# philres/ngmlr

Hardware: AMD Instinct MI355X
Metric: aligned Gbp/hour (PacBio 10kb synthetic, convex-gap SW hot path, host buffers in -> results out, CIGAR bit-exact) (higher is better)
Workload: dtype f32

## Files before the change

### ngmlr_amd/csrc/cvx_host_logic.h

```cpp
#ifndef CVX_HOST_LOGIC_H
#define CVX_HOST_LOGIC_H

#include <algorithm>
#include <atomic>
#include <cmath>
#include <condition_variable>
#include <cstdlib>
#include <cstring>
#include <deque>
#include <functional>
#include <mutex>
#include <system_error>
#include <thread>
#include <vector>

#include <pthread.h>

#include "cvx_align.h"
#include "cvx_types.h"

namespace cvx {


struct KernelClass {
// ... 700 lines not shown
				continue;
			}
		} else {
			ring = kClasses[k].ring();
		}
		r.ring = (int32_t) ring;
		r.r0 = p.r0;
		r.nsteps = p.rend - p.r0;
		r.dir_off = hp.dir_dwords;
		hp.dir_dwords += (uint64_t) ((r.nsteps + 31) / 32) * (uint64_t) r.ring * 2ull;
		r.mnw = k < 0 ? 0 : kClasses[k].m;
		if (k < 0) { hp.generic.push_back(i); continue; }
		hp.n_fast++;
		hp.cls[(size_t) k * 2 + (wrap ? 1 : 0)].push_back(i);
	}
	for (size_t slot = 0; slot < per_tile.size(); ++slot) {
		size_t deepest = 0;
		for (auto &v : per_tile[slot]) deepest = std::max(deepest, v.size());
		for (size_t g = 0; g < deepest; ++g)
			for (auto &v : per_tile[slot])
				if (g < v.size()) hp.chain_tasks[slot].push_back(v[g]);
	}
	for (auto &v : hp.cls) lpt_sort(v, plan);
}



struct ScheduleTuning {
	int exact_steps = kExactDirectSteps;
	int bt_group = 0;
	bool bt_per_class = true;
	bool overlap_post = false;
	int wide_prio = 1, gang_prio = 0, chain_prio = -1, chain_lds_kb = 48;
};

enum { kModeTwoPhase = 0, kModeExact = 1, kModeChain = 2 };

enum StreamSlot { kOnSide0 = 0, kOnPost = 1, kOnMain = 2, kOnSide1 = 3, kStreamSlots = 4 };

struct WalkPlan { int n_long = 0, long_lanes = 32, bulk_lanes = 64; };

inline WalkPlan walk_plan(int count, int n_walk, int bt_group, uint64_t mean_h, const int32_t *list, const TileIn *tin) {
	const int auto_group = count <= 6144 ? 64 : count <= 12288 ? 32 : count <= 49152 ? 16 : 8;
	WalkPlan w;
	w.bulk_lanes = bt_group > 0 ? bt_group : bt_group < 0 ? (n_walk < 4096 ? 64 : 8) : auto_group;
	if (bt_group <= 0 && w.bulk_lanes <= 16)
		while (w.n_long < count && (uint64_t) tin[(size_t) list[w.n_long]].H > 3 * mean_h) w.n_long++;
	return w;
}

inline size_t chain_pad_lds(uint64_t live, int num_cus, int chain_lds_kb, bool rings_beside) {
	const uint64_t resident = std::min<uint64_t>(8192, std::max<uint64_t>(768, live + live / 2 + 256));
	const size_t per_cu = (size_t) ((resident + (uint64_t) num_cus - 1) / (uint64_t) num_cus);
	size_t pad_lds = per_cu >= 32 ? 0 : (size_t) (160 * 1024) / per_cu - 4096;
	pad_lds = std::min<size_t>(pad_lds, 60 * 1024) / 256 * 256;
	if (rings_beside && chain_lds_kb > 0 && per_cu > 0 && per_cu < 32) {
		const size_t budget = (size_t) chain_lds_kb * 1024 / per_cu;
		const size_t capped = budget > 4096 ? (budget - 4096) / 256 * 256 : 0;
		pad_lds = std::min(pad_lds, capped);
	}
	return pad_lds;
}

struct FillLaunch {
	int kind = 0;
	int m = 0, gang = 1, wrap = 0;
	int slot = 0;
	const std::vector<int32_t> *tiles = nullptr;
	size_t list_off = 0;
	int n_direct = 0, count = 0;
	size_t pad_lds = 0;
	int prio = 0;
	int stream = kOnMain;
	size_t bt_off = 0;
	int bt_count = 0;
	WalkPlan walk;
	cvx_launch_info info;
};

struct ComputeSchedule {
	std::vector<FillLaunch> launches;
	size_t n_listed = 0;
	size_t bt_begin = 0;
	int n_walk = 0;
	bool per_class = false;
	WalkPlan walk;
	size_t chain_task_off[kNumChainClasses * 2] = {0}, chain_tile_off[kNumChainClasses * 2] = {0};
	size_t chain_blk_off = 0, chain_bytes = 0;
};

inline void build_schedule(HostPlan &hp, const TilePlan *plan, const TileIn *tin, int n, uint64_t n_rows, int num_cus,
		const ScheduleTuning &t, int32_t *lists, ComputeSchedule &s) {
	size_t n_listed = 0;
	size_t cls_off[kNumClasses * 2];
	int n_direct[kNumClasses * 2];
	int ring_classes = 0;
	for (size_t c = 0; c < hp.cls.size(); ++c) {
		std::vector<int32_t> &v = hp.cls[c];
		cls_off[c] = n_listed;
		n_direct[c] = 0;
		if (v.empty()) continue;
		ring_classes++;
		auto direct = [&](int32_t ti) { return hp.trun[(size_t) ti].nsteps >= t.exact_steps; };
		const int nl = t.exact_steps > 0 ? (int) std::count_if(v.begin(), v.end(), direct) : 0;
		if (nl > 0 && nl <= kExactDirectMaxTiles) {
			std::stable_partition(v.begin(), v.end(), direct);
			for (int q = 0; q < nl; ++q) hp.tout[(size_t) v[(size_t) q]].pad = kPadRedo;
			n_direct[c] = nl;
		}
		memcpy(lists + n_listed, v.data(), v.size() * sizeof(int32_t));
		n_listed += v.size();
	}
	const size_t generic_begin = n_listed;
	if (!hp.generic.empty()) memcpy(lists + n_listed, hp.generic.data(), hp.generic.size() * sizeof(int32_t));
	n_listed += hp.generic.size();

	s.launches.clear();
	s.launches.reserve((size_t) (kNumChainClasses + kNumClasses) * 2 + 1);
	for (size_t c = 0; c < hp.chain_tasks.size(); ++c) {
		if (hp.chain_tasks[c].empty()) continue;
		FillLaunch L;
		L.kind = CVX_LAUNCH_CHAINED;
		L.m = kChainClasses[c / 2]; L.wrap = (int) (c & 1); L.slot = (int) c;
		L.tiles = &hp.chain_tiles[c];
		L.count = (int) hp.chain_tasks[c].size();
		L.prio = t.chain_prio >= 0 ? t.chain_prio : 1;
		uint64_t live = 0;
		for (int32_t ti : hp.chain_tiles[c]) live += (uint64_t) plan[(size_t) ti].need / (uint64_t) (64 * L.m + kChainChunk) + 2;
		L.pad_lds = chain_pad_lds(live, num_cus, t.chain_lds_kb, ring_classes > 0);
		s.launches.push_back(L);
	}
	bool widest = true;
	for (int cc = (int) hp.cls.size() - 1; cc >= 0; --cc) {
		const size_t c = (size_t) cc;
		if (hp.cls[c].empty()) continue;
		const KernelClass &kc = kClasses[c / 2];
		FillLaunch L;
		L.kind = kc.gang > 1 ? CVX_LAUNCH_GANG : CVX_LAUNCH_WHOLE;
		L.m = kc.m; L.gang = kc.gang; L.wrap = (int) (c & 1); L.slot = cc;
		L.tiles = &hp.cls[c];
		L.list_off = cls_off[c]; L.n_direct = n_direct[c]; L.count = (int) hp.cls[c].size();
		L.prio = kc.gang > 1 ? t.gang_prio : (widest && ring_classes > 1) ? t.wide_prio : 0;
		widest = false;
		s.launches.push_back(L);
	}
	if (!hp.generic.empty()) {
		FillLaunch L;
		L.kind = CVX_LAUNCH_CATCH_ALL;
		L.m = 0; L.gang = 16; L.wrap = 1;
		L.tiles = &hp.generic;
		L.list_off = generic_begin; L.count = (int) hp.generic.size();
		s.launches.push_back(L);
	}

	int order[kStreamSlots], n_order = 0;
	for (int sl = 0; sl < kStreamSlots; ++sl) if (sl != kOnPost || !t.overlap_post) order[n_order++] = sl;
	s.bt_begin = n_listed;
	constexpr int kBuckets = 4096;
	auto bucket = [&](int32_t ti) { const int k = tin[(size_t) ti].H >> 5; return kBuckets - 1 - (k < kBuckets ? k : kBuckets - 1); };
	std::vector<int32_t> count((size_t) kBuckets + 1);
	for (size_t i = 0; i < s.launches.size(); ++i) {
		FillLaunch &L = s.launches[i];
		L.stream = order[i % (size_t) n_order];
		memset(&L.info, 0, sizeof(L.info));
		L.info.slots_per_lane = L.m; L.info.wrap16 = L.wrap; L.info.n_tiles = (int) L.tiles->size(); L.info.kind = L.kind;
		L.info.waves = L.kind == CVX_LAUNCH_CHAINED ? L.count : L.gang;
		std::fill(count.begin(), count.end(), 0);
		for (int32_t ti : *L.tiles) {
			const TilePlan &p = plan[(size_t) ti];
			const TileIn &in = tin[(size_t) ti];
			L.info.cells += p.cells; L.info.active_cells += p.active;
			L.info.alg_bytes += p.cells + 6ull * (uint64_t) in.H + 2ull * (uint64_t) in.W;
			L.info.read_bases += (uint64_t) in.H;
			if (!hp.trun[(size_t) ti].skip) count[(size_t) bucket(ti) + 1]++;
		}
		for (int k = 0; k < kBuckets; ++k) count[(size_t) k + 1] += count[(size_t) k];
		L.bt_off = n_listed;
		L.bt_count = count[(size_t) kBuckets];
		for (int32_t ti : *L.tiles) if (!hp.trun[(size_t) ti].skip) lists[n_listed + (size_t) count[(size_t) bucket(ti)]++] = ti;
		n_listed += (size_t) L.bt_count;
	}
	s.n_listed = n_listed;
	s.n_walk = (int) (n_listed - s.bt_begin);

	s.per_class = t.bt_per_class && s.launches.size() > 1 && !t.overlap_post && s.n_walk >= 4096;
	const uint64_t mean_h = n_rows / (uint64_t) std::max(n, 1);
	if (s.per_class) for (FillLaunch &L : s.launches) L.walk = walk_plan(L.bt_count, s.n_walk, t.bt_group, mean_h, lists + L.bt_off, tin);
	else s.walk = walk_plan(s.n_walk, s.n_walk, t.bt_group, mean_h, lists + s.bt_begin, tin);

	s.chain_blk_off = s.chain_bytes = 0;
	if (hp.n_chained) {
		for (size_t c = 0; c < hp.chain_tasks.size(); ++c) { s.chain_task_off[c] = s.chain_bytes; s.chain_bytes += hp.chain_tasks[c].size() * sizeof(ChainTask); }
		s.chain_blk_off = s.chain_bytes; s.chain_bytes += hp.chain_blk.size() * sizeof(ChainBlk);
		for (size_t c = 0; c < hp.chain_tiles.size(); ++c) { s.chain_tile_off[c] = s.chain_bytes; s.chain_bytes += (hp.chain_tiles[c].size() * sizeof(int32_t) + 7) / 8 * 8; }
	}
}

}

#endif
```

### ngmlr_amd/csrc/cvx_rt.h

```cpp
#ifndef CVX_RT_H
#define CVX_RT_H

#include <hip/hip_runtime_api.h>

#include <atomic>
#include <cstdint>
#include <mutex>
#include <string>
#include <vector>

#include "cvx_align.h"
#include "cvx_host_logic.h"
#include "cvx_launch.h"
#include "cvx_nm_regions.h"
#include "cvx_rt_err.h"
#include "cvx_types.h"

using namespace cvx;

#define HIP_TRY(expr)                                                              \
	do {                                                                           \
		hipError_t e_ = (expr);                                                    \
		if (e_ != hipSuccess) {                                                    \
			set_err("%s failed: %s (%s:%d)", #expr, hipGetErrorString(e_), __FILE__, __LINE__); \
// ... 86 lines not shown
			want = asked;
			e = hipHostMalloc(&p, want, hipHostMallocDefault);
		}
		if (e != hipSuccess) {
			(void) hipGetLastError();
			set_err("hipHostMalloc(%zu bytes) failed: %s", want, hipGetErrorString(e));
			p = nullptr;
			return CVX_ERR_OOM;
		}
		cap = want;
		if (hwm && cap > *hwm) *hwm = cap;
		return CVX_OK;
	}
	void release() {
		if (p) (void) hipHostFree(p);
		p = nullptr;
		cap = 0;
	}
	template <typename T> T *as() const { return static_cast<T *>(p); }
};

bool in_pinned_block(const void *p, uint64_t bytes);
float ev_ms(hipEvent_t a, hipEvent_t b);
int ensure_streams(cvx_context *c);
void search_state_free(cvx_search_state *ss);
float search_kernel_ms(const cvx_search_state *ss);
float search_score_kernel_ms(const cvx_search_state *ss);
void score_state_free(cvx_score_state *ss);

}

static const int kAuxStreams = 2;

enum LaunchEvent { kLevStart = 0, kLevTwoPhase = 1, kLevExact = 2, kLevWalked = 3, kLevPerLaunch = 4 };

enum BatchState { kFailed = -1, kEmpty = 0, kUploaded = 1, kPlanned = 2, kComputed = 3, kFinished = 4 };

struct cvx_batch_s {
	int n = 0;
	int state = kEmpty;
	bool in_flight = false;
	hipStream_t s_run = nullptr;
	int fail_rc = CVX_OK;
	std::string fail_msg;
	uint64_t seq_total = 0, n_rows = 0, n_rowsx = 0;
	uint64_t zero_copy_bytes = 0;
	uint64_t ops_total = 0;
	uint64_t dense_cap = 0;
	bool have_ops = false;

	PinBuf h_zero;
	size_t zero_cap = 0;
	PinBuf h_seq, h_delta, h_rsrc, h_rowsx, h_tin;
	std::vector<RowDesc> chain_rows;
	PinBuf h_plan;
	PinBuf h_trun, h_tout, h_lists, h_goff;
	PinBuf h_res;
	PinBuf h_ops;

	DevBuf<uint8_t> d_seq;
	DevBuf<RowDesc> d_rows;
	DevBuf<uint8_t> d_delta;
	DevBuf<RowSrc> d_rsrc;
	DevBuf<RowDesc> d_rowsx;
	DevBuf<TileIn> d_tin;
	DevBuf<TilePlan> d_plan;
	DevBuf<TileRun> d_trun;
// ... 14 lines not shown
	DevBuf<uint8_t> d_text;
	bool text_done = false;
	DevBuf<unsigned long long> d_nmoff;
	DevBuf<int32_t> d_nm;
	PinBuf h_nmoff;
	PinBuf h_nm;
	hipEvent_t ev_nm0 = nullptr, ev_nm1 = nullptr;
	DevBuf<unsigned long long> d_nmroff;
	DevBuf<NmOpen> d_nmopen;
	DevBuf<NmRegion> d_nmstage;
	DevBuf<NmRegion> d_nmreg;
	PinBuf h_nmroff, h_nmopen;
	PinBuf h_nmreg;
	PinBuf h_win;
	PinBuf h_refs;
	uint64_t refs_base = 0;
	bool have_refs = false;
	DevBuf<WindowDesc> d_win;
	PinBuf h_reads;
	PinBuf h_segs;
	DevBuf<uint8_t> d_reads, d_segs;
	PinBuf h_chain;
	DevBuf<uint8_t> d_chain;
	DevBuf<BoundaryRec> d_bnd;
	uint32_t bnd_epoch = 0;
	DevBuf<ChainOut> d_chain_out;

	hipEvent_t ev_bt0 = nullptr, ev_bt1 = nullptr;
	hipEvent_t ev_in = nullptr;
	hipEvent_t ev_res = nullptr;
	hipEvent_t ev[5] = {nullptr, nullptr, nullptr, nullptr, nullptr};
	std::vector<hipEvent_t> lev;
	std::vector<cvx_launch_info> launches;
	cvx_timing timing;

	const TileIn *tin() const { return h_tin.as<TileIn>(); }
	const TilePlan *plan() const { return h_plan.as<TilePlan>(); }
	const ResultRec *res() const { return h_res.as<ResultRec>(); }
	const BatchSummary *summary() const { return reinterpret_cast<const BatchSummary *>(h_res.as<uint8_t>() + (size_t) n * sizeof(ResultRec)); }

	static const int kSharedMarks = 40;
	void bind(size_t *marks) {
		int k = 0;
		PinBuf *pins[] = { &h_seq, &h_delta, &h_rsrc, &h_tin, &h_plan, &h_trun, &h_tout, &h_lists, &h_res, &h_ops, &h_chain };
		for (PinBuf *b_ : pins) b_->hwm = &marks[k++];
		d_seq.hwm = &marks[k++]; d_rows.hwm = &marks[k++]; d_delta.hwm = &marks[k++]; d_rsrc.hwm = &marks[k++]; d_tin.hwm = &marks[k++];
		d_plan.hwm = &marks[k++]; d_trun.hwm = &marks[k++]; d_tout.hwm = &marks[k++]; d_dirs.hwm = &marks[k++]; d_regions.hwm = &marks[k++];
		d_lists.hwm = &marks[k++]; d_dstoff.hwm = &marks[k++]; d_dense.hwm = &marks[k++]; d_res.hwm = &marks[k++];
		d_chain.hwm = &marks[k++]; d_bnd.hwm = &marks[k++]; d_chain_out.hwm = &marks[k++];
		h_text.hwm = &marks[k++]; h_nm.hwm = &marks[k++]; d_text.hwm = &marks[k++]; d_nm.hwm = &marks[k++];
		h_reads.hwm = &marks[k++]; h_segs.hwm = &marks[k++]; d_reads.hwm = &marks[k++]; d_segs.hwm = &marks[k++];
		static_assert(11 + 17 + 4 + 4 <= kSharedMarks, "marks");
	}
	int make_events() {
		if (!ev_in) HIP_TRY(hipEventCreateWithFlags(&ev_in, hipEventDisableTiming));
		if (!ev_res) HIP_TRY(hipEventCreateWithFlags(&ev_res, hipEventDisableTiming));
		if (!ev_bt0) HIP_TRY(hipEventCreateWithFlags(&ev_bt0, hipEventDisableTiming));
		if (!ev_bt1) HIP_TRY(hipEventCreateWithFlags(&ev_bt1, hipEventDisableTiming));
		for (auto &e : ev) if (!e) HIP_TRY(hipEventCreate(&e));
		return CVX_OK;
	}
	void release() {
		h_zero.release(); zero_cap = 0;
		h_seq.release(); h_delta.release(); h_rsrc.release(); h_rowsx.release(); h_tin.release();
		d_delta.release(); d_rsrc.release(); d_rowsx.release(); h_plan.release(); h_trun.release(); h_tout.release();
		h_lists.release(); h_goff.release(); h_res.release(); h_ops.release();
		d_seq.release(); d_rows.release(); d_tin.release(); d_plan.release(); d_trun.release();
		d_tout.release(); d_dirs.release(); d_regions.release(); d_lists.release();
		d_counters.release(); d_dstoff.release(); d_dense.release(); d_res.release();
		d_gscratch.release(); d_gscratch_off.release();
		h_win.release(); d_win.release(); h_refs.release();
		h_reads.release(); h_segs.release(); d_reads.release(); d_segs.release();
		h_ext.release(); h_trec.release(); h_toff.release(); h_text.release();
		d_ext.release(); d_trec.release(); d_tlen.release(); d_text.release();
		d_nmoff.release(); d_nm.release(); h_nmoff.release(); h_nm.release();
		d_nmroff.release(); d_nmopen.release(); d_nmstage.release(); d_nmreg.release(); h_nmroff.release(); h_nmopen.release(); h_nmreg.release();
		if (ev_nm0) { (void) hipEventDestroy(ev_nm0); ev_nm0 = nullptr; }
		if (ev_nm1) { (void) hipEventDestroy(ev_nm1); ev_nm1 = nullptr; }
		h_chain.release(); d_chain.release(); d_bnd.release(); d_chain_out.release();
		if (ev_in) { (void) hipEventDestroy(ev_in); ev_in = nullptr; }
		if (ev_res) { (void) hipEventDestroy(ev_res); ev_res = nullptr; }
		if (ev_bt0) { (void) hipEventDestroy(ev_bt0); ev_bt0 = nullptr; }
		if (ev_bt1) { (void) hipEventDestroy(ev_bt1); ev_bt1 = nullptr; }
		for (auto &e : ev) if (e) { (void) hipEventDestroy(e); e = nullptr; }
		for (auto &e : lev) if (e) (void) hipEventDestroy(e);
		lev.clear();
	}
};

struct cvx_context {
	int device = 0;
	hipStream_t s_io = nullptr;
	hipStream_t s_main = nullptr;
	hipStream_t s_text = nullptr;
	hipStream_t s_post = nullptr;
	hipStream_t aux[kAuxStreams] = {nullptr};
	bool service = false;
	bool owns_main = true;
	std::mutex streams_mtx;
	std::atomic<bool> streams_ready{false};
	hipStream_t s_main2 = nullptr, s_post2 = nullptr, aux2[kAuxStreams] = {nullptr};
	unsigned small_jobs = 0;
	ScoreParams sp;
	uint64_t max_matrix_mb = 10000;
	int num_cus = 256;
	int pack_threads = 16;
	int tune_min_slots = 0;
	int tune_late_min = kLateMinGroups;
	int tune_late_shift = kLateShift;
	int tune_max_slots = 0;
	int tune_long_need = 0;
	int tune_gang_prio = 0;
	int tune_gangs = 0;
	int tune_long_steps = 0, tune_small_batch = 0;
	bool single_lane = true;
	int tune_exact_steps = kExactDirectSteps;
	int tune_wide_prio = 1;
	int tune_chain_prio = -1;
	int tune_chain_lds_kb = 48;
	int tune_chain_m = 0;
	int tune_force_wrap = 0;
	int tune_pen_table = 1;
	int test_fail_compute = 0;
	int bt_group = 0;
	bool bt_per_class = true;
	bool overlap_post = false;
	bool scalar_twin = false;
	bool force_generic = false;
	bool sse_variant = false;
	size_t marks[cvx_batch_s::kSharedMarks] = {0};
	std::vector<cvx_batch_s *> pool;
	std::vector<cvx_batch_s *> pending;
	std::vector<cvx_batch_s *> live;
	float segments_kernel_ms = 0.0f;
	float decode_kernel_ms = 0.0f;
	bool score_no_diag = false;
	struct cvx_score_state *score = nullptr;
	struct cvx_search_state *search = nullptr;
};

struct cvx_genome_s {
	int device = 0;
	uint64_t n_nibbles = 0;
	int32_t n_starts = 0;
	DevBuf<uint8_t> d_bin;
	DevBuf<uint64_t> d_starts;
};

#endif
```

### ngmlr_amd/csrc/cvx_rt_align.cpp

```cpp
#include <algorithm>
#include <atomic>
#include <chrono>
#include <cstdio>
#include <cstdlib>
#include <cstring>
#include <new>
#include <string>
#include <vector>

#include "cvx_qry_stage.h"
#include "cvx_rt.h"

namespace {

struct SegmentsIn {
	int32_t n_reads;
	const uint8_t *arena;
	const uint64_t *offsets;
	const cvx_read_segment *qry;
};

static const size_t kPoolBatches = 8;

cvx_batch_s *acquire_batch(cvx_context *h) {
	if (!h->pool.empty()) {
		cvx_batch_s *b = h->pool.back();
		h->pool.pop_back();
		return b;
	}
	return new (std::nothrow) cvx_batch_s();
}

void recycle_batch(cvx_context *h, cvx_batch_s *b) {
	const bool failed = b->state == kFailed;
	b->state = kEmpty;
	b->in_flight = false;
	b->have_ops = false;
	b->have_refs = false;
	b->text_done = false;
	b->fail_rc = CVX_OK;
	b->fail_msg.clear();
	if (h) {
// ... 236 lines not shown
		if (!hp.chain_tasks[c].empty()) memcpy(hc + sch.chain_task_off[c], hp.chain_tasks[c].data(), hp.chain_tasks[c].size() * sizeof(ChainTask));
	memcpy(hc + sch.chain_blk_off, hp.chain_blk.data(), hp.chain_blk.size() * sizeof(ChainBlk));
	for (size_t c = 0; c < hp.chain_tiles.size(); ++c)
		if (!hp.chain_tiles[c].empty()) memcpy(hc + sch.chain_tile_off[c], hp.chain_tiles[c].data(), hp.chain_tiles[c].size() * sizeof(int32_t));
	RC_TRY(b->d_chain.ensure(sch.chain_bytes));
	RC_TRY(b->d_chain_out.ensure(hp.chain_blk.size()));
	{
		const size_t had = b->d_bnd.cap;
		RC_TRY(b->d_bnd.ensure((size_t) hp.bnd_recs + 64));
		if (b->d_bnd.cap != had || b->bnd_epoch >= kBndEpochMax) {
			HIP_TRY(hipMemsetAsync(b->d_bnd.p, 0, b->d_bnd.cap * sizeof(BoundaryRec), st));
			b->bnd_epoch = 0;
		}
		b->bnd_epoch += 1;
	}
	HIP_TRY(hipMemcpyAsync(b->d_chain.p, hc, sch.chain_bytes, hipMemcpyHostToDevice, st));
	return CVX_OK;
}

int stage_compute(cvx_context *h, cvx_batch_s *b, bool streaming = false) {
	const int n = b->n;
	if (h->test_fail_compute > 0 && --h->test_fail_compute == 0) {
		set_err("stage_compute: failure injected by CVX_TUNE_FAIL_COMPUTE");
		return CVX_ERR_OOM;
	}
	const bool second = streaming && n > 0 && n < kSmallJobTiles && !h->single_lane && ((h->small_jobs++ & 1u) != 0u);
	hipStream_t const S_main = second ? h->s_main2 : h->s_main;
	hipStream_t const S_post = second ? h->s_post2 : h->s_post;
	hipStream_t const *S_aux = second ? h->aux2 : h->aux;
	b->s_run = S_main;
	hipStream_t st = S_main;
	HIP_TRY(hipEventSynchronize(b->ev_in));
	b->launches.clear();
	b->ops_total = 0;
	b->have_ops = false;
	if (n == 0) {
		HIP_TRY(hipEventRecord(b->ev[4], st));
		hipStream_t ps = h->overlap_post ? S_post : S_main;
		HIP_TRY(hipStreamWaitEvent(ps, b->ev[4], 0));
		HIP_TRY(hipEventRecord(b->ev[2], ps));
		HIP_TRY(hipEventRecord(b->ev[3], ps));
		HIP_TRY(hipEventRecord(b->ev_res, ps));
		b->state = kComputed;
		return CVX_OK;
	}

	HostPlan hp;
	PlanTuning tune;
	tune.min_slots = h->tune_min_slots; tune.max_slots = h->tune_max_slots; tune.force_wrap = h->tune_force_wrap; tune.chain_m = h->tune_chain_m;
	tune.force_generic = h->force_generic ? 1 : 0;
	tune.long_steps = h->tune_long_steps; tune.small_batch = h->tune_small_batch; tune.long_need = h->tune_long_need;
	tune.no_gangs = h->tune_gangs ? 0 : 1;
	const RowSrc *rsrc = b->h_rsrc.as<RowSrc>();
	host_plan_rows(n, b->plan(), b->tin(), [&](int i, std::vector<RowDesc> &tmp) -> const RowDesc * {
		tmp.resize((size_t) std::max(b->tin()[(size_t) i].H, 1));
		expand_rows_host(rsrc[(size_t) i], b->tin()[(size_t) i].H, b->h_delta.as<uint8_t>(), b->h_rowsx.as<RowDesc>(), tmp.data());
		return tmp.data();
	}, true, tune, hp);
	const std::vector<int32_t> &generic = hp.generic;
	RC_TRY(b->d_dirs.ensure((size_t) hp.dir_dwords + 64));
	RC_TRY(b->d_regions.ensure((size_t) hp.ops_ints + 64));
	b->dense_cap = std::min<uint64_t>(hp.ops_ints, hp.ops_ints / 3 + 64ull * (uint64_t) n);
	RC_TRY(b->d_dense.ensure((size_t) b->dense_cap + 64));
	b->dense_cap = std::max<uint64_t>(b->dense_cap, b->d_dense.cap - 64);

	RC_TRY(b->h_trun.ensure((size_t) n * sizeof(TileRun)));
	RC_TRY(b->h_tout.ensure((size_t) n * sizeof(TileOut)));
	RC_TRY(b->h_lists.ensure((size_t) 2 * n * sizeof(int32_t) + 64));
	ScheduleTuning stune;
	stune.exact_steps = h->tune_exact_steps; stune.bt_group = h->bt_group; stune.bt_per_class = h->bt_per_class; stune.overlap_post = h->overlap_post;
	stune.wide_prio = h->tune_wide_prio; stune.gang_prio = h->tune_gang_prio; stune.chain_prio = h->tune_chain_prio; stune.chain_lds_kb = h->tune_chain_lds_kb;
	ComputeSchedule sch;
	build_schedule(hp, b->plan(), b->tin(), n, b->n_rows, h->num_cus, stune, b->h_lists.as<int32_t>(), sch);
	memcpy(b->h_trun.p, hp.trun.data(), (size_t) n * sizeof(TileRun));
	memcpy(b->h_tout.p, hp.tout.data(), (size_t) n * sizeof(TileOut));
	if (!generic.empty()) {
		RC_TRY(b->h_goff.ensure((generic.size() + 1) * sizeof(uint64_t)));
		uint64_t *goff = b->h_goff.as<uint64_t>();
		goff[0] = 0;
		for (size_t g = 0; g < generic.size(); ++g)
			goff[g + 1] = goff[g] + (uint64_t) generic_scratch_bytes(hp.trun[(size_t) generic[g]].ring);
		RC_TRY(b->d_gscratch.ensure((size_t) goff[generic.size()] + 256));
		RC_TRY(b->d_gscratch_off.ensure(generic.size() + 1));
		HIP_TRY(hipMemcpyAsync(b->d_gscratch_off.p, goff, (generic.size() + 1) * sizeof(uint64_t), hipMemcpyHostToDevice, st));
	}
	if (hp.n_chained) RC_TRY(upload_chain(b, hp, sch, st));
	HIP_TRY(hipMemcpyAsync(b->d_trun.p, b->h_trun.p, (size_t) n * sizeof(TileRun), hipMemcpyHostToDevice, st));
	HIP_TRY(hipMemcpyAsync(b->d_tout.p, b->h_tout.p, (size_t) n * sizeof(TileOut), hipMemcpyHostToDevice, st));
	if (sch.n_listed) HIP_TRY(hipMemcpyAsync(b->d_lists.p, b->h_lists.p, sch.n_listed * sizeof(int32_t), hipMemcpyHostToDevice, st));
	HIP_TRY(hipEventRecord(b->ev[4], st));

	FillArgs fa;
	BacktrackArgs ba;
	kernel_args(h, b, hp.n_chained ? reinterpret_cast<const ChainBlk *>(b->d_chain.p + sch.chain_blk_off) : nullptr, fa, ba);
	static_assert(kAuxStreams == 2, "StreamSlot names two side streams");
	hipStream_t fill_streams[kStreamSlots];
	fill_streams[kOnSide0] = S_aux[0]; fill_streams[kOnPost] = S_post; fill_streams[kOnMain] = st; fill_streams[kOnSide1] = S_aux[1];
	const int launches = (int) sch.launches.size();
	while (b->lev.size() < (size_t) launches * kLevPerLaunch) {
		hipEvent_t e;
		HIP_TRY(hipEventCreate(&e));
		b->lev.push_back(e);
	}
	for (int i = 0; i < launches; ++i) {
		const FillLaunch &L = sch.launches[(size_t) i];
		const hipStream_t ls = fill_streams[L.stream];
		const hipEvent_t *le = &b->lev[(size_t) i * kLevPerLaunch];
		const bool wrap = L.wrap != 0;
		b->launches.push_back(L.info);
		HIP_TRY(hipStreamWaitEvent(ls, b->ev[4], 0));
		HIP_TRY(hipEventRecord(le[kLevStart], ls));
		FillArgs a = fa;
		a.chain_prio = L.prio;
		if (L.kind == CVX_LAUNCH_CHAINED) {
			a.list_n = L.count;
			a.tasks = reinterpret_cast<const ChainTask *>(b->d_chain.p + sch.chain_task_off[L.slot]);
			a.chain_ticket = b->d_counters.p + 8 + L.slot;
			a.bnd = b->d_bnd.p;
			a.bnd_epoch = b->bnd_epoch;
			a.chain_out = b->d_chain_out.p;
			HIP_TRY(launch_fill(L.m, 1, wrap, kModeChain, a, L.pad_lds, ls));
			HIP_TRY(launch_chain_reduce(reinterpret_cast<const int32_t *>(b->d_chain.p + sch.chain_tile_off[L.slot]), L.info.n_tiles,
					b->d_trun.p, b->d_chain_out.p, b->d_tout.p, ls));
			HIP_TRY(hipEventRecord(le[kLevTwoPhase], ls));
		} else if (L.kind == CVX_LAUNCH_CATCH_ALL) {
			a.list = b->d_lists.p + L.list_off;
			a.list_n = L.count;
			HIP_TRY(launch_fill_generic(a, h->sse_variant, b->d_gscratch.p, b->d_gscratch_off.p, ls));
			HIP_TRY(hipEventRecord(le[kLevTwoPhase], ls));
		} else {
			a.list = b->d_lists.p + L.list_off;
			a.list_n = L.n_direct;
			if (a.list_n > 0) HIP_TRY(launch_fill(L.m, L.gang, wrap, kModeExact, a, 0, ls));
			a.list += L.n_direct;
			a.list_n = L.count - L.n_direct;
			if (a.list_n > 0) HIP_TRY(launch_fill(L.m, L.gang, wrap, kModeTwoPhase, a, 0, ls));
			HIP_TRY(hipEventRecord(le[kLevTwoPhase], ls));
			if (a.list_n > 0) HIP_TRY(launch_fill(L.m, L.gang, wrap, kModeExact, a, 0, ls));
		}
		HIP_TRY(hipEventRecord(le[kLevExact], ls));
		if (sch.per_class) RC_TRY(issue_walk(b, ba, L.walk, L.bt_off, L.bt_count, ls, nullptr));
		HIP_TRY(hipEventRecord(le[kLevWalked], ls));
	}
	st = h->overlap_post ? S_post : S_main;
	HIP_TRY(hipStreamWaitEvent(st, b->ev[4], 0));
	for (int i = 0; i < launches; ++i) HIP_TRY(hipStreamWaitEvent(st, b->lev[(size_t) i * kLevPerLaunch + kLevWalked], 0));
	HIP_TRY(hipEventRecord(b->ev[2], st));

	if (!sch.per_class) RC_TRY(issue_walk(b, ba, sch.walk, sch.bt_begin, sch.n_walk, st, S_aux[0]));
	ResultRec *d_rec = reinterpret_cast<ResultRec *>(b->d_res.p);
	BatchSummary *d_sum = reinterpret_cast<BatchSummary *>(b->d_res.p + (size_t) n * sizeof(ResultRec));
	HIP_TRY(launch_finalize(b->d_tout.p, b->d_plan.p, b->d_dstoff.p, b->d_dstoff.p + n, d_rec, d_sum, b->d_counters.p, n, b->dense_cap, st));
	HIP_TRY(launch_compact(b->d_regions.p, b->d_trun.p, b->d_tout.p, b->d_dstoff.p, b->d_dense.p, n, b->dense_cap, st));
	HIP_TRY(hipEventRecord(b->ev[3], st));
	HIP_TRY(hipMemcpyAsync(b->h_res.p, b->d_res.p, (size_t) n * sizeof(ResultRec) + sizeof(BatchSummary), hipMemcpyDeviceToHost, st));
	HIP_TRY(hipEventRecord(b->ev_res, st));

	b->timing.cells = hp.cells;
	b->timing.active_cells = hp.active;
	b->timing.dir_bytes = hp.dir_dwords * 4;
	b->timing.n_fill_launches = launches;
	b->timing.n_tiles_fast = hp.n_fast;
	b->timing.n_tiles_chained = hp.n_chained;
	b->state = kComputed;
	return CVX_OK;
}

int stage_results(cvx_context *h, cvx_batch_s *b) {
	(void) h;
	if (b->state < kComputed) { set_err("internal: results requested from a batch whose kernels were never queued (state %d)", b->state); return CVX_ERR_ARG; }
	HIP_TRY(hipEventSynchronize(b->ev_res));
	if (b->n == 0) { b->ops_total = 0; b->state = kFinished; return CVX_OK; }
	const BatchSummary *s = b->summary();
	b->ops_total = s->ops_total;
	const int launches = b->timing.n_fill_launches;
	for (int i = 0; i < launches; ++i) b->launches[(size_t) i].ms = ev_ms(b->lev[(size_t) i * kLevPerLaunch + kLevStart], b->lev[(size_t) i * kLevPerLaunch + kLevTwoPhase]);
	b->timing.plan_ms = ev_ms(b->ev[0], b->ev[1]);
	float fill_end = 0.0f;
	for (int i = 0; i < launches; ++i) fill_end = std::max(fill_end, ev_ms(b->ev[4], b->lev[(size_t) i * kLevPerLaunch + kLevExact]));
	if (launches == 0) fill_end = ev_ms(b->ev[4], b->ev[2]);
	b->timing.fill_ms = fill_end;
	b->timing.backtrack_ms = std::max(0.0f, ev_ms(b->ev[4], b->ev[3]) - fill_end);
	b->timing.total_ms = b->timing.plan_ms + ev_ms(b->ev[4], b->ev[3]);
	b->timing.n_tiles_redone = s->n_redone;
	b->timing.chain_task_ticks = s->chain_task_ticks;
	b->timing.chain_poll_ticks = s->chain_poll_ticks;
	b->state = kFinished;
	return CVX_OK;
}

int stage_ops(cvx_context *h, cvx_batch_s *b) {
	if (b->have_ops) return CVX_OK;
	if (b->ops_total > b->dense_cap) {
		const uint64_t cap = b->ops_total;
		RC_TRY(b->d_dense.ensure((size_t) cap + 64));
		b->dense_cap = b->d_dense.cap - 64;
		hipStream_t ps = b->s_run ? b->s_run : h->s_main;
		HIP_TRY(launch_compact(b->d_regions.p, b->d_trun.p, b->d_tout.p, b->d_dstoff.p, b->d_dense.p, b->n, b->dense_cap, ps));
		HIP_TRY(hipStreamSynchronize(ps));
	}
	if (b->ops_total) {
		RC_TRY(b->h_ops.ensure((size_t) b->ops_total * sizeof(uint32_t)));
		HIP_TRY(hipMemcpyAsync(b->h_ops.p, b->d_dense.p, (size_t) b->ops_total * sizeof(uint32_t), hipMemcpyDeviceToHost, h->s_io));
		HIP_TRY(hipStreamSynchronize(h->s_io));
	}
	b->have_ops = true;
	return CVX_OK;
}

int pump(cvx_context *h, bool block, const cvx_batch_s *upto) {
	while (!h->pending.empty()) {
		cvx_batch_s *b = h->pending.front();
// ... 426 lines not shown
```

### ngmlr_amd/csrc/cvx_runtime.cpp

```cpp
#include <hip/hip_runtime_api.h>
#include <dirent.h>
#include <unistd.h>

#include <algorithm>
#include <atomic>
#include <cmath>
#include <cstdarg>
#include <cstdio>
#include <cstdlib>
#include <cstring>
#include <functional>
#include <mutex>
#include <new>
#include <string>
#include <vector>

#include "cvx_rt.h"

namespace {

static const int kServiceStreamsMax = 16, kMaxServiceDevices = 64;
struct ServiceStreams { hipStream_t st[kServiceStreamsMax] = {nullptr}; unsigned next = 0; };
ServiceStreams g_service_streams[kMaxServiceDevices];
std::mutex g_service_mtx;
// ... 20 lines not shown

bool in_pinned_block(const void *p, uint64_t bytes) {
	const char *c = static_cast<const char *>(p);
	std::lock_guard<std::mutex> lk(g_pin_mtx);
	for (const auto &b : g_pin_blocks)
		if (c >= b.first && c + bytes <= b.first + b.second) return true;
	return false;
}

float ev_ms(hipEvent_t a, hipEvent_t b) {
	float ms = 0.0f;
	if (hipEventElapsedTime(&ms, a, b) != hipSuccess) { (void) hipGetLastError(); return 0.0f; }
	return ms;
}

int ensure_streams(cvx_context *c) {
	if (c->streams_ready.load(std::memory_order_acquire)) return CVX_OK;
	std::lock_guard<std::mutex> lk(c->streams_mtx);
	if (c->streams_ready.load(std::memory_order_relaxed)) return CVX_OK;
	int prio_lo = 0, prio_hi = 0;
	(void) hipDeviceGetStreamPriorityRange(&prio_lo, &prio_hi);
	hipError_t e = hipSuccess;
	auto make = [&](hipStream_t *st) { if (e == hipSuccess && *st == nullptr) e = hipStreamCreateWithFlags(st, hipStreamNonBlocking); };
	make(&c->s_post);
	{
		const char *tp = getenv("CVX_TEXT_STREAM_PRIO");
		if (e == hipSuccess && c->s_text == nullptr && !(tp && atoi(tp) == 0)) e = hipStreamCreateWithPriority(&c->s_text, hipStreamNonBlocking, prio_hi);
	}
	make(&c->s_text);
	for (int i = 0; i < kAuxStreams; ++i) make(&c->aux[i]);
	make(&c->s_main2);
	make(&c->s_post2);
	for (int i = 0; i < kAuxStreams; ++i) make(&c->aux2[i]);
	if (e == hipSuccess) e = hipStreamCreateWithPriority(&c->s_io, hipStreamNonBlocking, prio_hi);
	if (e != hipSuccess) { set_err("hipStreamCreate failed: %s", hipGetErrorString(e)); return CVX_ERR_HIP; }
	c->streams_ready.store(true, std::memory_order_release);
	return CVX_OK;
}

}

namespace cvx {
void pack_pool_run(int n_tasks, const std::function<void(int)> &fn) { PackPool::get().run(n_tasks, fn); }
}

static int g_hwq_set_by_library = 0;
static std::atomic<int> g_blocking_sync[64];
static int g_runtime_up_at_load = 0;
__attribute__((constructor)) static void cvx_process_settings() {
	g_hwq_set_by_library = getenv("GPU_MAX_HW_QUEUES") == nullptr;
	if (DIR *d = opendir("/proc/self/fd")) {
		while (struct dirent *e = readdir(d)) {
			char path[320], target[64];
			snprintf(path, sizeof(path), "/proc/self/fd/%s", e->d_name);
			const ssize_t n = readlink(path, target, sizeof(target) - 1);
			if (n > 0) { target[n] = 0; if (strcmp(target, "/dev/kfd") == 0) { g_runtime_up_at_load = 1; break; } }
		}
		closedir(d);
	}
	setenv("GPU_MAX_HW_QUEUES", "16", 0);
}

extern "C" {

const char *cvx_last_error(void) { return g_err.c_str(); }

// ... 82 lines not shown
		std::call_once(once[device_id & 63], [&] {
			if (g_runtime_up_at_load && g_hwq_set_by_library)
				fprintf(stderr, "cvx_create: a HIP runtime was already initialised when libcvxalign.so was loaded: GPU_MAX_HW_QUEUES=16 came too late for it -- "
						"export it before the process starts, or mixed launches run their fill classes one after the other (cvx_runtime_regime)\n");
			const char *w = getenv("CVX_WAIT");
			if (w && strcmp(w, "spin") == 0) { g_blocking_sync[device_id & 63] = 3; return; }
			const hipError_t fe = hipSetDeviceFlags(hipDeviceScheduleBlockingSync);
			g_blocking_sync[device_id & 63] = fe == hipSuccess ? 1 : 2;
			if (fe != hipSuccess) {
				(void) hipGetLastError();
				fprintf(stderr, "cvx_create: device %d stays in its current scheduling mode (%s): host threads that wait for it will spin\n", device_id, hipGetErrorString(fe));
			}
		});
	}
	hipDeviceProp_t prop;
	HIP_TRY(hipGetDeviceProperties(&prop, device_id));
	if (strncmp(prop.gcnArchName, "gfx950", 6) != 0) {
		set_err("cvx_create: device %d is %s; this library carries gfx950 code only", device_id, prop.gcnArchName);
		return CVX_ERR_NO_DEVICE;
	}
	cvx_context *c = new (std::nothrow) cvx_context();
	if (!c) return CVX_ERR_OOM;
	c->device = device_id;
	c->num_cus = prop.multiProcessorCount > 0 ? prop.multiProcessorCount : 256;
	c->sp.mat = p->match; c->sp.mis = p->mismatch; c->sp.go = p->gap_open;
	c->sp.ge = p->gap_extend; c->sp.gem = p->gap_extend_min; c->sp.decay = p->gap_decay;
	c->sp.misx = twin_mismatch_x(p->mismatch);
	c->scalar_twin = scalar_twin;
	c->max_matrix_mb = !sem.matrix_cap ? ~0ull : (max_matrix_mb ? max_matrix_mb : 10000);
	c->sse_variant = sem.sse_variant;
	if (const char *e = getenv("CVX_TUNE_BT_GROUP")) c->bt_group = atoi(e);
	if (const char *e = getenv("CVX_TUNE_BT_PER_CLASS")) c->bt_per_class = atoi(e) != 0;
	if (const char *e = getenv("CVX_TUNE_OVERLAP_POST")) c->overlap_post = atoi(e) != 0;
	if (const char *e = getenv("CVX_TUNE_SSE_VARIANT")) c->sse_variant = c->sse_variant || (atoi(e) != 0 && !scalar_twin);
	c->force_generic = sem.force_generic || c->sse_variant;
	c->pack_threads = PackPool::get().size();
	if (const char *e = getenv("CVX_TUNE_MIN_M")) c->tune_min_slots = atoi(e);
	if (const char *e = getenv("CVX_TUNE_FORCE_WRAP16")) c->tune_force_wrap = atoi(e);
	if (const char *e = getenv("CVX_TUNE_PEN_TABLE")) c->tune_pen_table = atoi(e) != 0;
	{
		volatile float prod = (float) kPenClamp * p->gap_decay;
		volatile float at_clamp = p->gap_extend + prod;
		const bool reached = !(at_clamp < p->gap_extend_min);
		if (!(p->gap_decay >= 0.0f) || !(reached || p->gap_decay == 0.0f)) c->tune_pen_table = 0;
	}
	if (const char *e = getenv("CVX_TUNE_FAIL_COMPUTE")) c->test_fail_compute = atoi(e);
	if (const char *e = getenv("CVX_TUNE_SCORE_NO_DIAG")) c->score_no_diag = atoi(e) != 0;
	if (const char *e = getenv("CVX_TUNE_MAX_M")) c->tune_max_slots = atoi(e);
	if (const char *e = getenv("CVX_TUNE_CHAIN_M")) c->tune_chain_m = atoi(e);
	if (const char *e = getenv("CVX_TUNE_CHAIN_PRIO")) c->tune_chain_prio = atoi(e) != 0;
	if (const char *e = getenv("CVX_TUNE_CHAIN_LDS_KB")) c->tune_chain_lds_kb = atoi(e) > 0 ? atoi(e) : 0;
	if (const char *e = getenv("CVX_TUNE_WIDE_PRIO")) c->tune_wide_prio = atoi(e);
	if (const char *e = getenv("CVX_TUNE_EXACT_STEPS")) c->tune_exact_steps = atoi(e);
	if (const char *e = getenv("CVX_TUNE_TWO_LANES")) c->single_lane = atoi(e) == 0;
	if (const char *e = getenv("CVX_TUNE_LONG_STEPS")) c->tune_long_steps = atoi(e);
	if (const char *e = getenv("CVX_TUNE_SMALL_BATCH")) c->tune_small_batch = atoi(e);
	if (const char *e = getenv("CVX_TUNE_LONG_NEED")) c->tune_long_need = atoi(e);
	if (const char *e = getenv("CVX_TUNE_GANGS")) c->tune_gangs = atoi(e) != 0 && !sem.no_gangs;
	if (const char *e = getenv("CVX_TUNE_GANG_PRIO")) c->tune_gang_prio = atoi(e) != 0;
	if (const char *e = getenv("CVX_TUNE_LATE_MIN")) c->tune_late_min = std::max(1, atoi(e));
	if (const char *e = getenv("CVX_TUNE_LATE_SHIFT")) c->tune_late_shift = std::min(16, std::max(0, atoi(e)));
	hipError_t e = hipSuccess;
	c->service = (flags & CVX_CREATE_SERVICE) != 0;
	const char *sp = getenv("CVX_SERVICE_PRIO");
	int shared = 4;
	if (const char *e2 = getenv("CVX_SERVICE_STREAMS")) shared = atoi(e2) > 0 ? std::min(atoi(e2), kServiceStreamsMax) : 0;
// ... 5 lines not shown
		c->s_main = ss.st[k];
		c->owns_main = false;
	} else if (c->service && sp && atoi(sp) != 0) {
		int prio_lo = 0, prio_hi = 0;
		(void) hipDeviceGetStreamPriorityRange(&prio_lo, &prio_hi);
		e = hipStreamCreateWithPriority(&c->s_main, hipStreamNonBlocking, prio_hi);
	} else {
		e = hipStreamCreateWithFlags(&c->s_main, hipStreamNonBlocking);
	}
	if (e != hipSuccess) {
		set_err("hipStreamCreate failed: %s", hipGetErrorString(e));
		cvx_destroy(c);
		return CVX_ERR_HIP;
	}
	*out = c;
	return CVX_OK;
	ABI_GUARD_END
}

void cvx_destroy(cvx_handle h) {
	ABI_GUARD_BEGIN
	if (!h) return;
	(void) hipSetDevice(h->device);
	(void) hipDeviceSynchronize();
	g_deferred.drain();
	if (h->s_main && h->owns_main) (void) hipStreamDestroy(h->s_main);
	if (h->s_post) (void) hipStreamDestroy(h->s_post);
	if (h->s_text) (void) hipStreamDestroy(h->s_text);
	if (h->s_io) (void) hipStreamDestroy(h->s_io);
	for (auto &a : h->aux) if (a) (void) hipStreamDestroy(a);
	if (h->s_main2) (void) hipStreamDestroy(h->s_main2);
	if (h->s_post2) (void) hipStreamDestroy(h->s_post2);
	for (auto &a : h->aux2) if (a) (void) hipStreamDestroy(a);
	for (cvx_batch_s *b : h->pool) { b->release(); delete b; }
	h->pool.clear();
	for (cvx_batch_s *b : h->live) { b->release(); delete b; }
	h->live.clear();
	h->pending.clear();
	score_state_free(h->score);
	search_state_free(h->search);
	delete h;
	ABI_GUARD_END_VOID
}


int cvx_host_alloc(uint64_t bytes, void **out) {
	ABI_GUARD_BEGIN
	if (!out) { set_err("cvx_host_alloc: NULL argument"); return CVX_ERR_ARG; }
	*out = nullptr;
	int ndev = 0;
	if (hipGetDeviceCount(&ndev) != hipSuccess || ndev <= 0) { (void) hipGetLastError(); set_err("cvx_host_alloc: no HIP device"); return CVX_ERR_NO_DEVICE; }
	void *p = nullptr;
	const size_t want = (size_t) bytes + 4096;
	hipError_t e = hipHostMalloc(&p, want, hipHostMallocPortable);
	if (e != hipSuccess) { (void) hipGetLastError(); set_err("hipHostMalloc(%zu bytes) failed: %s", want, hipGetErrorString(e)); return CVX_ERR_OOM; }
	{
		std::lock_guard<std::mutex> lk(g_pin_mtx);
		g_pin_blocks.emplace_back(static_cast<const char *>(p), want);
	}
	*out = p;
	return CVX_OK;
	ABI_GUARD_END
}

void cvx_host_free(void *p) {
	ABI_GUARD_BEGIN
// ... 12 lines not shown
```

Baseline: 16200.

## Split the tail of each ring fill launch onto a separate low-priority stream

For non-gang ring classes, the last few tiles of each two-phase fill launch are peeled off. Their count is sized from queried kernel occupancy, about one residency round. They are launched on a dedicated low-priority tail stream that starts together with the head, and the tail's backtrack walk waits on the tail's exact pass. The goal is to fill the CU idle time during the last partial wave of a large launch by overlapping the tail with the head. It adds a stream, more events, split bucket sorting and per-class walk plans, and it depends on the low-priority stream existing (prio_lo > 0).

```diff
diff --git a/ngmlr_amd/csrc/cvx_fill_occupancy.h b/ngmlr_amd/csrc/cvx_fill_occupancy.h
--- /dev/null
+++ b/ngmlr_amd/csrc/cvx_fill_occupancy.h
@@ -0,0 +1,10 @@
+#ifndef CVX_FILL_OCCUPANCY_H
+#define CVX_FILL_OCCUPANCY_H
+
+namespace cvx {
+
+int fill_two_phase_waves_per_simd(int m, bool wrap, bool pen_table, bool twin);
+
+}
+
+#endif
diff --git a/ngmlr_amd/csrc/cvx_fill_occupancy.hip b/ngmlr_amd/csrc/cvx_fill_occupancy.hip
--- /dev/null
+++ b/ngmlr_amd/csrc/cvx_fill_occupancy.hip
@@ -0,0 +1,40 @@
+#include <hip/hip_runtime.h>
+
+#include "cvx_types.h"
+#include "cvx_fill_occupancy.h"
+
+namespace cvx {
+
+enum { kOccTwoPhase = 0 };
+
+template <int M, bool WRAP, int MODE, bool TAB, int G> __global__ void fill_ring_kernel(const FillArgs a);
+template <int M, bool WRAP, int MODE, bool TAB, int G> __global__ void fill_ring_twin_kernel(const FillArgs a);
+
+template <typename K>
+static int waves_per_simd(K kernel) {
+	int blocks = 0;
+	if (hipOccupancyMaxActiveBlocksPerMultiprocessor(&blocks, kernel, 64, 0) != hipSuccess) { (void) hipGetLastError(); return -1; }
+	return blocks > 0 ? blocks / 4 : -1;
+}
+
+template <int M, bool WRAP>
+static int two_phase_t(bool pen_table, bool twin) {
+	if (twin) {
+		if (!WRAP && pen_table) return waves_per_simd(fill_ring_twin_kernel<M, false, kOccTwoPhase, true, 1>);
+		return waves_per_simd(fill_ring_twin_kernel<M, WRAP, kOccTwoPhase, false, 1>);
+	}
+	if (!WRAP && pen_table) return waves_per_simd(fill_ring_kernel<M, false, kOccTwoPhase, true, 1>);
+	return waves_per_simd(fill_ring_kernel<M, WRAP, kOccTwoPhase, false, 1>);
+}
+
+int fill_two_phase_waves_per_simd(int m, bool wrap, bool pen_table, bool twin) {
+	switch (m) {
+	case 1: return wrap ? two_phase_t<1, true>(pen_table, twin) : two_phase_t<1, false>(pen_table, twin);
+	case 2: return wrap ? two_phase_t<2, true>(pen_table, twin) : two_phase_t<2, false>(pen_table, twin);
+	case 3: return wrap ? two_phase_t<3, true>(pen_table, twin) : two_phase_t<3, false>(pen_table, twin);
+	case 4: return wrap ? two_phase_t<4, true>(pen_table, twin) : two_phase_t<4, false>(pen_table, twin);
+	default: return -1;
+	}
+}
+
+}
diff --git a/ngmlr_amd/csrc/cvx_host_logic.h b/ngmlr_amd/csrc/cvx_host_logic.h
--- a/ngmlr_amd/csrc/cvx_host_logic.h
+++ b/ngmlr_amd/csrc/cvx_host_logic.h
@@ -756,7 +756,25 @@
 	bool bt_per_class = true;
 	bool overlap_post = false;
 	int wide_prio = 1, gang_prio = 0, chain_prio = -1, chain_lds_kb = 48;
-};
+	int tail_tiles = 0;
+	float tail_rounds = 1.0f;
+	int tail_waves_per_simd[kNumClasses * 2] = {0};
+};
+
+enum { kTailAuto = -1 };
+static const int kTailMinRounds = 4;
+static const int kTailMinWalk = 4096;
+
+inline int tail_split(const ScheduleTuning &t, int cls, int gang, int two_phase, int n_walk, int num_cus) {
+	if (t.tail_tiles == 0 || gang > 1 || t.overlap_post || !t.bt_per_class) return 0;
+	int tail = t.tail_tiles;
+	if (t.tail_tiles == kTailAuto) {
+		const int64_t resident = (int64_t) num_cus * 4 * (int64_t) t.tail_waves_per_simd[cls];
+		if (resident <= 0 || (int64_t) two_phase < kTailMinRounds * resident || n_walk < kTailMinWalk) return 0;
+		tail = (int) ((double) t.tail_rounds * (double) resident + 0.5);
+	}
+	return (tail > 0 && tail < two_phase) ? tail : 0;
+}
 
 enum { kModeTwoPhase = 0, kModeExact = 1, kModeChain = 2 };
 
@@ -796,9 +814,12 @@
 	size_t pad_lds = 0;
 	int prio = 0;
 	int stream = kOnMain;
+	int tail_count = 0;
 	size_t bt_off = 0;
 	int bt_count = 0;
+	int bt_tail_count = 0;
 	WalkPlan walk;
+	WalkPlan walk_tail;
 	cvx_launch_info info;
 };
 
@@ -835,6 +856,8 @@
 		memcpy(lists + n_listed, v.data(), v.size() * sizeof(int32_t));
 		n_listed += v.size();
 	}
+	int n_computed = 0;
+	for (int i = 0; i < n; ++i) if (!hp.trun[(size_t) i].skip) n_computed++;
 	const size_t generic_begin = n_listed;
 	if (!hp.generic.empty()) memcpy(lists + n_listed, hp.generic.data(), hp.generic.size() * sizeof(int32_t));
 	n_listed += hp.generic.size();
@@ -866,6 +889,7 @@
 		L.list_off = cls_off[c]; L.n_direct = n_direct[c]; L.count = (int) hp.cls[c].size();
 		L.prio = kc.gang > 1 ? t.gang_prio : (widest && ring_classes > 1) ? t.wide_prio : 0;
 		widest = false;
+		L.tail_count = tail_split(t, cc, kc.gang, L.count - L.n_direct, n_computed, num_cus);
 		s.launches.push_back(L);
 	}
 	if (!hp.generic.empty()) {
@@ -883,33 +907,45 @@
 	constexpr int kBuckets = 4096;
 	auto bucket = [&](int32_t ti) { const int k = tin[(size_t) ti].H >> 5; return kBuckets - 1 - (k < kBuckets ? k : kBuckets - 1); };
 	std::vector<int32_t> count((size_t) kBuckets + 1);
+	bool any_split = false;
 	for (size_t i = 0; i < s.launches.size(); ++i) {
 		FillLaunch &L = s.launches[i];
 		L.stream = order[i % (size_t) n_order];
 		memset(&L.info, 0, sizeof(L.info));
 		L.info.slots_per_lane = L.m; L.info.wrap16 = L.wrap; L.info.n_tiles = (int) L.tiles->size(); L.info.kind = L.kind;
 		L.info.waves = L.kind == CVX_LAUNCH_CHAINED ? L.count : L.gang;
-		std::fill(count.begin(), count.end(), 0);
 		for (int32_t ti : *L.tiles) {
 			const TilePlan &p = plan[(size_t) ti];
 			const TileIn &in = tin[(size_t) ti];
 			L.info.cells += p.cells; L.info.active_cells += p.active;
 			L.info.alg_bytes += p.cells + 6ull * (uint64_t) in.H + 2ull * (uint64_t) in.W;
 			L.info.read_bases += (uint64_t) in.H;
-			if (!hp.trun[(size_t) ti].skip) count[(size_t) bucket(ti) + 1]++;
-		}
-		for (int k = 0; k < kBuckets; ++k) count[(size_t) k + 1] += count[(size_t) k];
+		}
 		L.bt_off = n_listed;
-		L.bt_count = count[(size_t) kBuckets];
-		for (int32_t ti : *L.tiles) if (!hp.trun[(size_t) ti].skip) lists[n_listed + (size_t) count[(size_t) bucket(ti)]++] = ti;
-		n_listed += (size_t) L.bt_count;
+		const size_t n_head = L.tiles->size() - (size_t) L.tail_count;
+		for (int part = 0; part < (L.tail_count > 0 ? 2 : 1); ++part) {
+			const int32_t *tb = L.tiles->data() + (part ? n_head : 0), *te = L.tiles->data() + (part ? L.tiles->size() : n_head);
+			std::fill(count.begin(), count.end(), 0);
+			for (const int32_t *q = tb; q < te; ++q) if (!hp.trun[(size_t) *q].skip) count[(size_t) bucket(*q) + 1]++;
+			for (int k = 0; k < kBuckets; ++k) count[(size_t) k + 1] += count[(size_t) k];
+			const int part_count = count[(size_t) kBuckets];
+			for (const int32_t *q = tb; q < te; ++q) if (!hp.trun[(size_t) *q].skip) lists[n_listed + (size_t) count[(size_t) bucket(*q)]++] = *q;
+			n_listed += (size_t) part_count;
+			if (part) L.bt_tail_count = part_count;
+		}
+		L.bt_count = (int) (n_listed - L.bt_off);
+		any_split = any_split || L.tail_count > 0;
 	}
 	s.n_listed = n_listed;
 	s.n_walk = (int) (n_listed - s.bt_begin);
 
-	s.per_class = t.bt_per_class && s.launches.size() > 1 && !t.overlap_post && s.n_walk >= 4096;
+	s.per_class = (t.bt_per_class && s.launches.size() > 1 && !t.overlap_post && s.n_walk >= 4096) || any_split;
 	const uint64_t mean_h = n_rows / (uint64_t) std::max(n, 1);
-	if (s.per_class) for (FillLaunch &L : s.launches) L.walk = walk_plan(L.bt_count, s.n_walk, t.bt_group, mean_h, lists + L.bt_off, tin);
+	if (s.per_class) for (FillLaunch &L : s.launches) {
+		const int n_head = L.bt_count - L.bt_tail_count;
+		L.walk = walk_plan(n_head, s.n_walk, t.bt_group, mean_h, lists + L.bt_off, tin);
+		if (L.bt_tail_count > 0) L.walk_tail = walk_plan(L.bt_tail_count, s.n_walk, t.bt_group, mean_h, lists + L.bt_off + (size_t) n_head, tin);
+	}
 	else s.walk = walk_plan(s.n_walk, s.n_walk, t.bt_group, mean_h, lists + s.bt_begin, tin);
 
 	s.chain_blk_off = s.chain_bytes = 0;
diff --git a/ngmlr_amd/csrc/cvx_rt.h b/ngmlr_amd/csrc/cvx_rt.h
--- a/ngmlr_amd/csrc/cvx_rt.h
+++ b/ngmlr_amd/csrc/cvx_rt.h
@@ -142,7 +142,7 @@
 
 static const int kAuxStreams = 2;
 
-enum LaunchEvent { kLevStart = 0, kLevTwoPhase = 1, kLevExact = 2, kLevWalked = 3, kLevPerLaunch = 4 };
+enum LaunchEvent { kLevStart = 0, kLevTwoPhase = 1, kLevExact = 2, kLevWalked = 3, kLevTailStart = 4, kLevTailTwoPhase = 5, kLevTailExact = 6, kLevPerLaunch = 7 };
 
 enum BatchState { kFailed = -1, kEmpty = 0, kUploaded = 1, kPlanned = 2, kComputed = 3, kFinished = 4 };
 
@@ -223,6 +223,7 @@
 	hipEvent_t ev[5] = {nullptr, nullptr, nullptr, nullptr, nullptr};
 	std::vector<hipEvent_t> lev;
 	std::vector<cvx_launch_info> launches;
+	std::vector<int> launch_tail;
 	cvx_timing timing;
 
 	const TileIn *tin() const { return h_tin.as<TileIn>(); }
@@ -286,6 +287,7 @@
 	hipStream_t s_text = nullptr;
 	hipStream_t s_post = nullptr;
 	hipStream_t aux[kAuxStreams] = {nullptr};
+	hipStream_t s_tail = nullptr;
 	bool service = false;
 	bool owns_main = true;
 	std::mutex streams_mtx;
@@ -314,6 +316,11 @@
 	int tune_pen_table = 1;
 	int test_fail_compute = 0;
 	int bt_group = 0;
+	int tail_split = cvx::kTailAuto;
+	float tail_rounds = 1.0f;
+	int tail_gate = 1;
+	int tail_trace = 0;
+	int fill_waves[cvx::kNumClasses * 2] = {0};
 	bool bt_per_class = true;
 	bool overlap_post = false;
 	bool scalar_twin = false;
diff --git a/ngmlr_amd/csrc/cvx_rt_align.cpp b/ngmlr_amd/csrc/cvx_rt_align.cpp
--- a/ngmlr_amd/csrc/cvx_rt_align.cpp
+++ b/ngmlr_amd/csrc/cvx_rt_align.cpp
@@ -8,6 +8,7 @@
 #include <string>
 #include <vector>
 
+#include "cvx_fill_occupancy.h"
 #include "cvx_qry_stage.h"
 #include "cvx_rt.h"
 
@@ -310,6 +311,7 @@
 	hipStream_t st = S_main;
 	HIP_TRY(hipEventSynchronize(b->ev_in));
 	b->launches.clear();
+	b->launch_tail.clear();
 	b->ops_total = 0;
 	b->have_ops = false;
 	if (n == 0) {
@@ -348,6 +350,15 @@
 	ScheduleTuning stune;
 	stune.exact_steps = h->tune_exact_steps; stune.bt_group = h->bt_group; stune.bt_per_class = h->bt_per_class; stune.overlap_post = h->overlap_post;
 	stune.wide_prio = h->tune_wide_prio; stune.gang_prio = h->tune_gang_prio; stune.chain_prio = h->tune_chain_prio; stune.chain_lds_kb = h->tune_chain_lds_kb;
+	stune.tail_tiles = h->s_tail ? h->tail_split : 0;
+	stune.tail_rounds = h->tail_rounds;
+	if (stune.tail_tiles == kTailAuto) {
+		for (size_t c = 0; c < hp.cls.size(); ++c) {
+			if (hp.cls[c].empty() || kClasses[c / 2].gang > 1) continue;
+			if (h->fill_waves[c] == 0) h->fill_waves[c] = fill_two_phase_waves_per_simd(kClasses[c / 2].m, (c & 1) != 0, h->tune_pen_table != 0, h->scalar_twin);
+			stune.tail_waves_per_simd[c] = std::max(0, h->fill_waves[c]);
+		}
+	}
 	ComputeSchedule sch;
 	build_schedule(hp, b->plan(), b->tin(), n, b->n_rows, h->num_cus, stune, b->h_lists.as<int32_t>(), sch);
 	memcpy(b->h_trun.p, hp.trun.data(), (size_t) n * sizeof(TileRun));
@@ -386,6 +397,7 @@
 		const hipEvent_t *le = &b->lev[(size_t) i * kLevPerLaunch];
 		const bool wrap = L.wrap != 0;
 		b->launches.push_back(L.info);
+		b->launch_tail.push_back(L.tail_count);
 		HIP_TRY(hipStreamWaitEvent(ls, b->ev[4], 0));
 		HIP_TRY(hipEventRecord(le[kLevStart], ls));
 		FillArgs a = fa;
@@ -411,13 +423,31 @@
 			a.list_n = L.n_direct;
 			if (a.list_n > 0) HIP_TRY(launch_fill(L.m, L.gang, wrap, kModeExact, a, 0, ls));
 			a.list += L.n_direct;
-			a.list_n = L.count - L.n_direct;
+			a.list_n = L.count - L.n_direct - L.tail_count;
 			if (a.list_n > 0) HIP_TRY(launch_fill(L.m, L.gang, wrap, kModeTwoPhase, a, 0, ls));
 			HIP_TRY(hipEventRecord(le[kLevTwoPhase], ls));
 			if (a.list_n > 0) HIP_TRY(launch_fill(L.m, L.gang, wrap, kModeExact, a, 0, ls));
+			if (L.tail_count > 0) {
+				FillArgs ta = a;
+				ta.list = a.list + a.list_n;
+				ta.list_n = L.tail_count;
+				HIP_TRY(hipStreamWaitEvent(h->s_tail, h->tail_gate ? le[kLevStart] : b->ev[4], 0));
+				HIP_TRY(hipEventRecord(le[kLevTailStart], h->s_tail));
+				HIP_TRY(launch_fill(L.m, L.gang, wrap, kModeTwoPhase, ta, 0, h->s_tail));
+				HIP_TRY(hipEventRecord(le[kLevTailTwoPhase], h->s_tail));
+				HIP_TRY(launch_fill(L.m, L.gang, wrap, kModeExact, ta, 0, h->s_tail));
+				HIP_TRY(hipEventRecord(le[kLevTailExact], h->s_tail));
+			}
 		}
 		HIP_TRY(hipEventRecord(le[kLevExact], ls));
-		if (sch.per_class) RC_TRY(issue_walk(b, ba, L.walk, L.bt_off, L.bt_count, ls, nullptr));
+		if (sch.per_class) {
+			const int n_head = L.bt_count - L.bt_tail_count;
+			RC_TRY(issue_walk(b, ba, L.walk, L.bt_off, n_head, ls, nullptr));
+			if (L.tail_count > 0) {
+				HIP_TRY(hipStreamWaitEvent(ls, le[kLevTailExact], 0));
+				RC_TRY(issue_walk(b, ba, L.walk_tail, L.bt_off + (size_t) n_head, L.bt_tail_count, ls, nullptr));
+			}
+		}
 		HIP_TRY(hipEventRecord(le[kLevWalked], ls));
 	}
 	st = h->overlap_post ? S_post : S_main;
@@ -445,17 +475,31 @@
 }
 
 int stage_results(cvx_context *h, cvx_batch_s *b) {
-	(void) h;
 	if (b->state < kComputed) { set_err("internal: results requested from a batch whose kernels were never queued (state %d)", b->state); return CVX_ERR_ARG; }
 	HIP_TRY(hipEventSynchronize(b->ev_res));
 	if (b->n == 0) { b->ops_total = 0; b->state = kFinished; return CVX_OK; }
 	const BatchSummary *s = b->summary();
 	b->ops_total = s->ops_total;
 	const int launches = b->timing.n_fill_launches;
-	for (int i = 0; i < launches; ++i) b->launches[(size_t) i].ms = ev_ms(b->lev[(size_t) i * kLevPerLaunch + kLevStart], b->lev[(size_t) i * kLevPerLaunch + kLevTwoPhase]);
+	for (int i = 0; i < launches; ++i) {
+		const hipEvent_t *le = &b->lev[(size_t) i * kLevPerLaunch];
+		b->launches[(size_t) i].ms = ev_ms(le[kLevStart], le[kLevTwoPhase]);
+		if (b->launch_tail[(size_t) i] > 0) b->launches[(size_t) i].ms = std::max(b->launches[(size_t) i].ms, ev_ms(le[kLevStart], le[kLevTailTwoPhase]));
+	}
 	b->timing.plan_ms = ev_ms(b->ev[0], b->ev[1]);
 	float fill_end = 0.0f;
-	for (int i = 0; i < launches; ++i) fill_end = std::max(fill_end, ev_ms(b->ev[4], b->lev[(size_t) i * kLevPerLaunch + kLevExact]));
+	for (int i = 0; i < launches; ++i) {
+		const hipEvent_t *le = &b->lev[(size_t) i * kLevPerLaunch];
+		fill_end = std::max(fill_end, ev_ms(b->ev[4], le[kLevExact]));
+		if (b->launch_tail[(size_t) i] > 0) {
+			fill_end = std::max(fill_end, ev_ms(b->ev[4], le[kLevTailExact]));
+			if (h->tail_trace)
+				fprintf(stderr, "cvx tail split: launch %d m=%d tiles=%d tail=%d  head two-phase end %.3f exact end %.3f  tail start %.3f two-phase end %.3f exact end %.3f  walked %.3f ms after the launch's start\n",
+						i, b->launches[(size_t) i].slots_per_lane, b->launches[(size_t) i].n_tiles, b->launch_tail[(size_t) i],
+						ev_ms(le[kLevStart], le[kLevTwoPhase]), ev_ms(le[kLevStart], le[kLevExact]), ev_ms(le[kLevStart], le[kLevTailStart]),
+						ev_ms(le[kLevStart], le[kLevTailTwoPhase]), ev_ms(le[kLevStart], le[kLevTailExact]), ev_ms(le[kLevStart], le[kLevWalked]));
+		}
+	}
 	if (launches == 0) fill_end = ev_ms(b->ev[4], b->ev[2]);
 	b->timing.fill_ms = fill_end;
 	b->timing.backtrack_ms = std::max(0.0f, ev_ms(b->ev[4], b->ev[3]) - fill_end);
diff --git a/ngmlr_amd/csrc/cvx_runtime.cpp b/ngmlr_amd/csrc/cvx_runtime.cpp
--- a/ngmlr_amd/csrc/cvx_runtime.cpp
+++ b/ngmlr_amd/csrc/cvx_runtime.cpp
@@ -76,6 +76,7 @@
 	make(&c->s_main2);
 	make(&c->s_post2);
 	for (int i = 0; i < kAuxStreams; ++i) make(&c->aux2[i]);
+	if (e == hipSuccess && c->s_tail == nullptr && c->tail_split != 0 && prio_lo > 0) e = hipStreamCreateWithPriority(&c->s_tail, hipStreamNonBlocking, prio_lo);
 	if (e == hipSuccess) e = hipStreamCreateWithPriority(&c->s_io, hipStreamNonBlocking, prio_hi);
 	if (e != hipSuccess) { set_err("hipStreamCreate failed: %s", hipGetErrorString(e)); return CVX_ERR_HIP; }
 	c->streams_ready.store(true, std::memory_order_release);
@@ -224,6 +225,10 @@
 	if (const char *e = getenv("CVX_TUNE_BT_GROUP")) c->bt_group = atoi(e);
 	if (const char *e = getenv("CVX_TUNE_BT_PER_CLASS")) c->bt_per_class = atoi(e) != 0;
 	if (const char *e = getenv("CVX_TUNE_OVERLAP_POST")) c->overlap_post = atoi(e) != 0;
+	if (const char *e = getenv("CVX_TUNE_TAIL_SPLIT")) c->tail_split = std::max(0, atoi(e));
+	if (const char *e = getenv("CVX_TUNE_TAIL_ROUNDS")) c->tail_rounds = (float) std::max(0.0, atof(e));
+	if (const char *e = getenv("CVX_TUNE_TAIL_TRACE")) c->tail_trace = atoi(e);
+	if (const char *e = getenv("CVX_TUNE_TAIL_GATE")) c->tail_gate = atoi(e);
 	if (const char *e = getenv("CVX_TUNE_SSE_VARIANT")) c->sse_variant = c->sse_variant || (atoi(e) != 0 && !scalar_twin);
 	c->force_generic = sem.force_generic || c->sse_variant;
 	c->pack_threads = PackPool::get().size();
@@ -295,6 +300,7 @@
 	if (h->s_main2) (void) hipStreamDestroy(h->s_main2);
 	if (h->s_post2) (void) hipStreamDestroy(h->s_post2);
 	for (auto &a : h->aux2) if (a) (void) hipStreamDestroy(a);
+	if (h->s_tail) (void) hipStreamDestroy(h->s_tail);
 	for (cvx_batch_s *b : h->pool) { b->release(); delete b; }
 	h->pool.clear();
 	for (cvx_batch_s *b : h->live) { b->release(); delete b; }
```

Result: faster. 16880, median of 6 (+4.2%).
